# 4paradigm/OpenEmbedding

Measured on AMD Instinct MI355X. Metric: samples/sec DeepFM Criteo, higher is better.
Workload: dtype bf16; 1 GPU; model=deepfm-dim9, global_batch=4096, fields=26, dense_features=13, optimizer=adagrad, graph=True, prefetch=False, table=array, cache_mb=0, parallelism=single-gpu

## Files before the change

### openembedding_amd/models/ctr.py

```python

from __future__ import annotations

import math
from typing import List, Optional, Sequence

import torch
import torch.nn as nn

from ..ops import hip_available
from ..torch import CombinedEmbedding
from .criteo import CRITEO_FIELD_VOCABS, N_DENSE


class _FusedCTRHeadFn(torch.autograd.Function):

    @staticmethod
    def forward(ctx, e_all, dense, w, b, use_fm, out_bf16, pad32=False):
        from ..ops import require_hip
        ext = require_hip()
        wf = w.reshape(-1).contiguous()
        e_all = e_all.contiguous()
        dense = dense.contiguous()
        deep_in, partial, s = ext.ctr_head_fwd(
            e_all, dense, wf, b.reshape(-1).contiguous(), use_fm, out_bf16,
            pad32)
        ctx.save_for_backward(e_all, dense, wf, s)
        ctx.use_fm = use_fm
        return deep_in, partial

    @staticmethod
    def backward(ctx, d_deep_in, d_partial):
        from ..ops import require_hip
        ext = require_hip()
        e_all, dense, wf, s = ctx.saved_tensors
        de_all, d_dense, dw, db = ext.ctr_head_bwd(
            e_all, dense, wf, d_deep_in.contiguous(),
            d_partial.contiguous(), s, ctx.use_fm)
        return de_all, d_dense, dw.view(1, -1), db, None, None, None


class _FusedMLP3Fn(torch.autograd.Function):

    @staticmethod
    def forward(ctx, x0, partial, w1, b1, w2, b2, w3, b3, w4, b4, bufs):
        from ..ops import require_hip
        ext = require_hip()
        srcs = [w1, w2, w3]
        dsts = [bufs["w1p"], bufs["w2p"], bufs["w3p"]]
        trans = [False, False, False]
        if any(ctx.needs_input_grad) and bufs.get("grad_mode", True):
            srcs += [w3, w2, w1]
            dsts += [bufs["w3tp"], bufs["w2tp"], bufs["w1tp"]]
            trans += [True, True, True]
        ext.mlp3_pack_frag([w.contiguous() for w in srcs], dsts, trans)
        w4f = w4.reshape(-1).contiguous()
        out, a1, a2, a3 = ext.mlp3_fwd(x0, bufs["w1p"], b1, bufs["w2p"], b2,
                                       bufs["w3p"], b3, w4f, b4,
                                       None if partial is None
                                       else partial.contiguous(), frag=True)
        ctx.save_for_backward(x0, w1, w2, w3, w4f, a1, a2, a3)
        ctx.bufs = bufs
        ctx._params = (w1, b1, w2, b2, w3, b3, w4, b4)
        ctx._has_partial = partial is not None
        return out

    @staticmethod
    def backward(ctx, dout):
        from ..ops import require_hip
        ext = require_hip()
        x0, w1, w2, w3, w4f, a1, a2, a3 = ctx.saved_tensors
        bufs = ctx.bufs
        K0 = w1.shape[1]
        params = ctx._params
        prebound = all(p.grad is not None for p in params)
        bias_fused = (prebound
                      and params[1].grad.dtype == torch.bfloat16
                      and all(params[i].grad.is_contiguous()
                              for i in (1, 3, 5, 6)))
        bscratch = None
        if bias_fused:
            H0 = a1.shape[1]
            bscratch = bufs.get("bscratch")
            if bscratch is None or bscratch.numel() != 4 * H0 + 1:
                bscratch = torch.zeros(4 * H0 + 1, dtype=torch.float32,
                                       device=a1.device)
                bufs["bscratch"] = bscratch
        dx0, dz1, dz2, dz3 = ext.mlp3_bwd(
            dout.contiguous(), a1, a2, a3, w4f,
            bufs["w3tp"], bufs["w2tp"], bufs["w1tp"], bscratch, frag=True)
        def _d():
# ... 336 lines not shown
```

### openembedding_amd/ops/csrc/bindings.cpp

```cpp

#include <torch/extension.h>
#include <ATen/cuda/CUDAContext.h>
#include <c10/cuda/CUDAGuard.h>

#include <cstdint>
#include <tuple>
#include <vector>

typedef unsigned long long u64;
typedef int64_t i64;
typedef struct ihipStream_t* hipStream_t_;

extern "C" {
void emb_unique(const i64*, long, u64*, int*, long, int*, unsigned char*,
                i64*, i64*, int*, const i64*, int, hipStream_t_);
void emb_unique_indexed(const i64*, long, u64*, int*, long, int*,
                        unsigned char*, i64*, i64*, int*, const i64*, int,
                        int*, int*, int*, int*, int*, int*, int*, long, int*,
                        int*, hipStream_t_);
void emb_unique_indexed_assign(const i64*, long, u64*, int*, long, int*,
                               unsigned char*, i64*, i64*, int*, const i64*,
                               int, int*, int*, int*, int*, int*, int*, int*,
                               long, int*, int*, unsigned char*, long, long,
                               i64*, unsigned char*, hipStream_t_);
// ... 13 lines not shown
                               float*, long, const float*, hipStream_t_);
void emb_ht_lookup(u64*, int*, long, const i64*, long, int*, i64*, i64*,
                   unsigned char*, int, const int*, long, hipStream_t_);
void emb_ht_rehash(const u64*, const int*, long, u64*, int*, long,
                   hipStream_t_);
void emb_array_touch(unsigned char*, const i64*, long, long, long, i64*,
                     unsigned char*, const int*, hipStream_t_);
void emb_gather_init(float*, float*, long, long, const i64*,
                     const unsigned char*, const i64*, long, const i64*,
                     float*, int, float, float, float, u64, const float*,
                     const int*, hipStream_t_);
void emb_reduce_by_inverse(const i64*, const float*, long, long, float*, u64*,
                           long, hipStream_t_);
void emb_reduce_bags_by_inverse(const i64*, const float*, long, long,
                                const int*, const i64*, long, int, float*,
                                u64*, long, hipStream_t_);
void emb_pool_fwd(const float*, long, long, const i64*, long, const void*,
                  int, long, const i64*, long, int, float*, int*,
                  hipStream_t_);
void emb_pool_fwd_weighted(const float*, long, long, const i64*, long,
                           const void*, int, long, const i64*, long, int,
                           const float*, float*, int*, float*, hipStream_t_);
void emb_reduce_bags_weighted_by_inverse(const i64*, const float*, long, long,
                                         const int*, const float*,
                                         const float*, long, float*, u64*,
                                         long, hipStream_t_);
void emb_pool_wgrad(const float*, long, long, const i64*, long, const void*,
                    int, long, const float*, const int*, const float*,
                    const float*, const float*, long, int, float*,
                    hipStream_t_);
void emb_pool_lookup(const float*, long, long, const i64*, long, const i64*,
                     long, int, const float*, const u64*, const int*, long,
                     const unsigned char*, long, float*, hipStream_t_);
long emb_quant_stride(int, long);
void emb_quantize_rows(int, const float*, long, long, const i64*, void*,
                       long, hipStream_t_);
void emb_pool_lookup_q(int, const void*, long, long, const i64*, long,
                       const i64*, long, int, const float*, const u64*,
                       const int*, long, const unsigned char*, long, float*,
                       hipStream_t_);
void emb_gather_lookup_q(int, const void*, long, long, const i64*, long,
                         const u64*, const int*, long, const unsigned char*,
                         long, float*, hipStream_t_);
void emb_apply_optimizer(int, float*, float*, long, long, const i64*, long,
                         const float*, const u64*, const float*, const int*,
                         hipStream_t_);
void emb_ctr_head_fwd(const float*, const float*, const float*, const float*, long,
                      long, long, long, long, void*, float*, float*, int,
                      int, hipStream_t_);
void emb_ctr_head_bwd(const float*, const float*, const float*, const void*,
                      const float*, const float*, long, long, long, long,
                      long, float*, float*, float*, float*, int, int,
                      hipStream_t_);
void emb_mlp3_bias_bwd(const float*, const void*, const void*, const void*,
                       const void*, long, long, float*, void*, void*, void*,
                       void*, void*, int, int, hipStream_t_);
void emb_mlp3_wgrad(const void*, const void*, const void*, const void*,
                    const void*, const void*, long, long, long, long,
                    float*, void*, void*, void*, float*, long, hipStream_t_);
void emb_mlp3_pack(const void*, void*, long, long, long, long, int,
                   const void*, void*, long, long, long, long, int,
                   const void*, void*, long, long, long, long, int,
                   hipStream_t_);
void emb_bce_fwd(const float*, const float*, long, float*, hipStream_t_);
void emb_bce_bwd(const float*, const float*, long, const float*, float*,
                 hipStream_t_);
void emb_bucketize_pad(const i64*, long, const int*, long, long, i64*, int*,
                       int*, int*, int*, hipStream_t_);
void emb_mask_tail(i64*, float*, u64*, long, long, const int*, hipStream_t_);
void emb_mark_rows(const i64*, long, const unsigned char*, const int*,
                   const int*, int*, long, hipStream_t_);
long emb_delta_tile_rows();
long emb_delta_tiles(long);
void emb_delta_count(const int*, long, int, const int*, const unsigned char*,
                     int*, hipStream_t_);
void emb_delta_compact(const int*, long, int, const int*,
                       const unsigned char*, const int*, i64*, hipStream_t_);
void emb_delta_gather(const float*, const float*, long, long, long,
                      const i64*, long, long, const i64*, long, long, long,
                      const int*, i64*, float*, float*, hipStream_t_);
void emb_fault_in(const i64*, long, const int*, const u64*, const int*, long,
                  const float*, const float*, float*, float*, long, long,
                  const i64*, unsigned char*, int*, hipStream_t_);
void emb_spill_rows(const i64*, const i64*, long, const float*, const float*,
                    float*, float*, long, long, hipStream_t_);
void emb_gather_host(const i64*, long, const i64*, const u64*, const int*,
                     long, const float*, float*, long, hipStream_t_);
void emb_gather_pad(const float*, const u64*, long, const int*, long, float*,
                    hipStream_t_);
void emb_scatter_out(const float*, const i64*, long, const int*, long, float*,
                     hipStream_t_);
void emb_split_payload(const float*, long, long, const int*, float*, u64*,
                       hipStream_t_);
void emb_flat_step_scalars(float*, float, float, hipStream_t_);
void emb_flat_opt(int, void*, float*, float*, float*, void*,
                  const float*, long, int, float, float, float, float,
                  hipStream_t_);
void emb_flat_adagrad_f32(float*, float*, const float*, long, float, float,
                          hipStream_t_);
void emb_flat_adagrad_bf16(float*, float*, const void*, void*, long, float,
                           float, hipStream_t_);
void emb_cin_fwd(const float*, const float*, const void*, float*, long,
                 long, long, long, long, hipStream_t_);
void emb_cin_dw(const void*, const void*, const void*, float*, long, long,
                long, long, long, hipStream_t_);
void emb_cin_dx(const float*, const void*, const float*, const float*,
// ... 1092 lines not shown
    return send_p;
}

torch::Tensor scatter_out(torch::Tensor rows_recv, torch::Tensor inverse,
                          torch::Tensor pos_of, int64_t n_elems) {
    CHECK_GPU(rows_recv); CHECK_CONT(rows_recv); CHECK_CONT(inverse);
    CHECK_CONT(pos_of);
    TORCH_CHECK(rows_recv.dtype() == torch::kFloat32 &&
                pos_of.dtype() == torch::kInt32, "scatter_out dtypes");
    const c10::cuda::CUDAGuard guard(rows_recv.device());
    long dim = rows_recv.size(1);
    auto out = torch::empty({n_elems, dim}, rows_recv.options());
    emb_scatter_out(rows_recv.data_ptr<float>(), inverse.data_ptr<i64>(),
                    n_elems, pos_of.data_ptr<int>(), dim,
                    out.data_ptr<float>(), cur_stream());
    return out;
}

std::tuple<torch::Tensor, torch::Tensor> split_payload(torch::Tensor g2c,
                                                       OptTensor u_dev) {
    CHECK_GPU(g2c); CHECK_CONT(g2c);
    TORCH_CHECK(g2c.dtype() == torch::kFloat32, "split_payload dtype");
    const c10::cuda::CUDAGuard guard(g2c.device());
    long u = g2c.size(0);
    long dim = g2c.size(1) - 1;
    auto grads = torch::empty({u, dim}, g2c.options());
    auto counts = torch::empty({u}, g2c.options().dtype(torch::kInt64));
    emb_split_payload(g2c.data_ptr<float>(), u, dim, u_ptr(u_dev),
                      grads.data_ptr<float>(), (u64*)counts.data_ptr<i64>(),
                      cur_stream());
    return {grads, counts};
}


void apply_optimizer(int64_t opt, torch::Tensor weights, torch::Tensor state,
                     torch::Tensor slots, torch::Tensor grads,
                     torch::Tensor counts, std::vector<double> cfg,
                     OptTensor u_dev) {
    CHECK_GPU(weights); CHECK_CONT(weights); CHECK_CONT(grads);
    const c10::cuda::CUDAGuard guard(weights.device());
    long n = slots.numel();
    long dim = weights.size(1);
    long sd = state.numel() ? state.size(1) : 0;
    float c[7] = {0, 0, 0, 0, 0, 0, 0};
    for (size_t i = 0; i < cfg.size() && i < 7; ++i) c[i] = (float)cfg[i];
    emb_apply_optimizer((int)opt, weights.data_ptr<float>(),
                        sd ? state.data_ptr<float>() : nullptr, dim, sd,
                        slots.data_ptr<i64>(), n, grads.data_ptr<float>(),
                        (const u64*)counts.data_ptr<i64>(), c, u_ptr(u_dev),
                        cur_stream());
}


std::tuple<torch::Tensor, torch::Tensor, torch::Tensor> ctr_head_fwd(
    torch::Tensor e_all, torch::Tensor dense, torch::Tensor w,
    torch::Tensor bias, bool use_fm, bool out_bf16, bool pad32) {
    CHECK_GPU(e_all); CHECK_CONT(e_all); CHECK_CONT(dense); CHECK_CONT(w);
    const c10::cuda::CUDAGuard guard(e_all.device());
    long B = e_all.size(0), F = e_all.size(1), D1 = e_all.size(2);
    long dim = D1 - 1, nd = dense.size(1);
    TORCH_CHECK(D1 <= 128, "ctr_head: dim+1 must be <= 128");
    TORCH_CHECK(nd <= 32, "ctr_head: dense features must be <= 32");
    auto out_opts = e_all.options().dtype(out_bf16 ? torch::kBFloat16
                                                   : torch::kFloat32);
    long width = F * dim + nd;
    long stride = pad32 ? ((width + 31) / 32) * 32 : width;
    auto deep_in = torch::empty({B, stride}, out_opts);
    auto partial = torch::empty({B}, e_all.options());
    auto s_out = torch::empty({B, dim}, e_all.options());
    CHECK_CONT(bias);
    emb_ctr_head_fwd(e_all.data_ptr<float>(), dense.data_ptr<float>(),
                     w.data_ptr<float>(), bias.data_ptr<float>(), B, F, dim, nd,
                     stride, deep_in.data_ptr(), partial.data_ptr<float>(),
                     s_out.data_ptr<float>(),
                     use_fm ? 1 : 0, out_bf16 ? 1 : 0, cur_stream());
    return {deep_in, partial, s_out};
}

std::tuple<torch::Tensor, torch::Tensor, torch::Tensor, torch::Tensor>
ctr_head_bwd(torch::Tensor e_all, torch::Tensor dense, torch::Tensor w,
             torch::Tensor d_deep_in, torch::Tensor d_partial,
             torch::Tensor s_in, bool use_fm) {
    CHECK_GPU(e_all); CHECK_CONT(e_all); CHECK_CONT(d_deep_in);
    const c10::cuda::CUDAGuard guard(e_all.device());
    long B = e_all.size(0), F = e_all.size(1), D1 = e_all.size(2);
    long dim = D1 - 1, nd = dense.size(1);
    long stride = d_deep_in.size(1);
    bool out_bf16 = d_deep_in.dtype() == torch::kBFloat16;
    auto de_all = torch::empty_like(e_all);
    auto d_dense = torch::empty_like(dense);
    auto dw = torch::empty_like(w);
    auto db = torch::empty({1}, w.options());
    if (B == 0) { dw.zero_(); db.zero_(); }
    emb_ctr_head_bwd(e_all.data_ptr<float>(), dense.data_ptr<float>(),
                     w.data_ptr<float>(), d_deep_in.data_ptr(),
                     d_partial.data_ptr<float>(),
                     s_in.data_ptr<float>(), B, F, dim, nd, stride,
                     de_all.data_ptr<float>(), d_dense.data_ptr<float>(),
                     dw.data_ptr<float>(), db.data_ptr<float>(),
                     use_fm ? 1 : 0, out_bf16 ? 1 : 0, cur_stream());
    return {de_all, d_dense, dw, db};
}


void flat_adagrad(torch::Tensor param, torch::Tensor accum,
                  torch::Tensor grad, c10::optional<torch::Tensor> master,
                  double lr, double eps) {
    CHECK_GPU(param); CHECK_CONT(param); CHECK_CONT(accum); CHECK_CONT(grad);
    const c10::cuda::CUDAGuard guard(param.device());
    long n = param.numel();
    if (param.dtype() == torch::kFloat32) {
        emb_flat_adagrad_f32(param.data_ptr<float>(), accum.data_ptr<float>(),
                             grad.data_ptr<float>(), n, (float)lr, (float)eps,
                             cur_stream());
    } else {
        TORCH_CHECK(param.dtype() == torch::kBFloat16 && master.has_value(),
                    "bf16 flat_adagrad needs a float32 master tensor");
        emb_flat_adagrad_bf16(master->data_ptr<float>(),
                              accum.data_ptr<float>(), grad.data_ptr(),
                              param.data_ptr(), n, (float)lr, (float)eps,
                              cur_stream());
    }
}

void flat_step_scalars(torch::Tensor sc, double b1, double b2) {
    CHECK_GPU(sc); CHECK_CONT(sc);
    TORCH_CHECK(sc.numel() >= 3 && sc.dtype() == torch::kFloat32,
                "step scalars must be float32 [3]");
    const c10::cuda::CUDAGuard guard(sc.device());
    emb_flat_step_scalars(sc.data_ptr<float>(), (float)b1, (float)b2,
                          cur_stream());
}

void flat_opt(int64_t opt, torch::Tensor param, OptTensor master,
              OptTensor s1, OptTensor s2, torch::Tensor grad, OptTensor sc,
              double lr, double c0, double c1, double c2) {
    CHECK_GPU(param); CHECK_CONT(param); CHECK_CONT(grad);
    const c10::cuda::CUDAGuard guard(param.device());
    long n = param.numel();
    bool bf16 = param.dtype() == torch::kBFloat16;
    float* mp = nullptr;
    if (bf16) {
        TORCH_CHECK(master.has_value(), "bf16 flat_opt needs fp32 master");
        mp = master->data_ptr<float>();
    } else {
        TORCH_CHECK(param.dtype() == torch::kFloat32, "flat_opt dtype");
    }
    emb_flat_opt((int)opt, param.data_ptr(), mp,
                 s1.has_value() ? s1->data_ptr<float>() : nullptr,
                 s2.has_value() ? s2->data_ptr<float>() : nullptr,
                 grad.data_ptr(),
                 sc.has_value() ? sc->data_ptr<float>() : nullptr,
                 n, bf16 ? 1 : 0, (float)lr, (float)c0, (float)c1,
                 (float)c2, cur_stream());
// ... 399 lines not shown
          "flat read over a packed slab, keys -> fp32 rows in one launch",
          pybind11::arg("slab"), pybind11::arg("dim"), pybind11::arg("fmt"),
          pybind11::arg("keys"),
          pybind11::arg("tk") = pybind11::none(),
          pybind11::arg("tv") = pybind11::none(),
          pybind11::arg("valid") = pybind11::none(),
          pybind11::arg("shard_num") = 1);
    m.def("apply_optimizer", &apply_optimizer, "fused sparse optimizer step");
    m.def("mask_tail", &mask_tail,
          "zero the garbage tail of a bounded block (enables multi-block "
          "merge by concatenation)");
    m.def("mark_rows", &mark_rows,
          "delta checkpoints: row_epoch[slot] = *epoch_dev for the named "
          "rows (optional byte mask and device count)",
          pybind11::arg("slots"), pybind11::arg("mask") = pybind11::none(),
          pybind11::arg("u_dev") = pybind11::none(),
          pybind11::arg("epoch_dev"), pybind11::arg("row_epoch"));
    m.attr("DELTA_TILE_ROWS") = emb_delta_tile_rows();
    m.def("select_changed", &select_changed,
          "delta checkpoints: ascending slots of the live rows with "
          "row_epoch >= since -> (slots [R] with a -1 tail, n_dev int32[1])",
          pybind11::arg("row_epoch"), pybind11::arg("since"),
          pybind11::arg("nrows_dev") = pybind11::none(),
          pybind11::arg("valid") = pybind11::none());
    m.def("gather_rows_by_slot", &gather_rows_by_slot,
          "delta checkpoints: keys, weights and state of "
          "slots[start:start+count] into staging buffers",
          pybind11::arg("weights"), pybind11::arg("state"),
          pybind11::arg("slot_keys") = pybind11::none(),
          pybind11::arg("shard_num") = 1, pybind11::arg("shard_id") = 0,
          pybind11::arg("slots"), pybind11::arg("start"),
          pybind11::arg("count"), pybind11::arg("n_dev"),
          pybind11::arg("keys_out") = pybind11::none(),
          pybind11::arg("w_out") = pybind11::none(),
          pybind11::arg("s_out") = pybind11::none());
    m.def("fault_in", &fault_in,
          "tier v2: copy host-resident rows into fresh cache slots, "
          "clearing their lazy-init mask");
    m.def("spill_rows", &spill_rows,
          "tier v2: copy cache rows into the pinned host slab");
    m.def("gather_host", &gather_host,
          "tier v2: read-only host-row gather for cache misses");
    m.def("bucketize_pad", &bucketize_pad,
          "owner-bucketize unique keys into a fixed padded [world, cap] "
          "wire block (sync-free multi-rank route)");
    m.def("gather_pad", &gather_pad,
          "gather grads+counts payload into the padded send layout");
    m.def("scatter_out", &scatter_out,
          "padded pull: wire rows -> per-element output (fused dup scatter)");
    m.def("split_payload", &split_payload,
          "split owner-reduced payload into grads + int64 counts");
    m.def("ctr_head_fwd", &ctr_head_fwd,
          "fused CTR head fwd: deep_in assembly (+cast) + FM + first-order "
          "+ dense linear");
    m.def("ctr_head_bwd", &ctr_head_bwd, "fused CTR head backward");
    m.def("mlp3_bwd", &mlp3_bwd,
          "fused dgrad chain backward of the 3-layer MLP (optionally "
          "carrying the head wgrad/bias sums)",
          pybind11::arg("dout"), pybind11::arg("a1"), pybind11::arg("a2"),
          pybind11::arg("a3"), pybind11::arg("w4"), pybind11::arg("w3t"),
          pybind11::arg("w2t"), pybind11::arg("w1t"),
          pybind11::arg("bias_scratch") = pybind11::none(),
          pybind11::arg("bm") = 0, pybind11::arg("frag") = false);
    m.def("mlp3_pack", &mlp3_pack,
          "refresh three padded (or transposed) weight copies in one "
          "launch");
    m.def("mlp3_pack_frag", &mlp3_pack_frag,
          "write up to six fragment-major weight images (pads included) "
          "in one launch",
          pybind11::arg("srcs"), pybind11::arg("dsts"),
          pybind11::arg("trans"));
    m.def("mlp3_fwd", &mlp3_fwd,
          "fused 3-hidden-layer MLP forward (bf16 MFMA, bias+ReLU fused)",
          pybind11::arg("x0"), pybind11::arg("w1"), pybind11::arg("b1"),
          pybind11::arg("w2"), pybind11::arg("b2"), pybind11::arg("w3"),
          pybind11::arg("b3"), pybind11::arg("w4"), pybind11::arg("b4"),
          pybind11::arg("partial"), pybind11::arg("bm") = 0,
          pybind11::arg("frag") = false);
    m.def("mlp3_wgrad", &mlp3_wgrad,
          pybind11::arg("dz1"), pybind11::arg("dz2"), pybind11::arg("dz3"),
          pybind11::arg("x0"), pybind11::arg("a1"), pybind11::arg("a2"),
          pybind11::arg("scratch"), pybind11::arg("dw1"),
          pybind11::arg("dw2"), pybind11::arg("dw3"),
          pybind11::arg("bias_scratch") = pybind11::none(),
          pybind11::arg("m_split") = 0,
          "all three MLP weight grads in one MFMA launch (+= into bf16 "
          "grads via fp32 scratch)");
    m.def("mlp3_bias_bwd", &mlp3_bias_bwd,
          "MLP bias grads + head wgrad in one pass over the dz mirrors "
          "(with_dz=false when the fused wgrad carried the dz sums)",
          pybind11::arg("dout"), pybind11::arg("dz1"), pybind11::arg("dz2"),
          pybind11::arg("dz3"), pybind11::arg("a3"),
          pybind11::arg("scratch"), pybind11::arg("db1"),
          pybind11::arg("db2"), pybind11::arg("db3"), pybind11::arg("dw4"),
          pybind11::arg("db4"), pybind11::arg("with_dz") = true,
          pybind11::arg("with_head") = true);
    m.def("cin_fwd", &cin_fwd,
          "CIN layer forward: implicit outer-product MFMA GEMM");
    m.def("cin_dw", &cin_dw,
          "CIN weight grad: per-field split-K MFMA with on-the-fly operand");
    m.def("cin_dx", &cin_dx,
          "CIN input grads: P=W^T dZ GEMM fused with the xk/x0 contractions");
    m.def("bce_fwd", &bce_fwd, "fused BCE-with-logits forward (mean)");
    m.def("bce_bwd", &bce_bwd, "fused BCE-with-logits backward");
    m.def("flat_adagrad", &flat_adagrad,
          "fused flat-buffer Adagrad (f32, or bf16 weights + f32 master)");
    m.def("flat_opt", &flat_opt,
          "fused flat-buffer dense optimizer (0=sgd, 1=adagrad, 2=adam)");
// ... 5 lines not shown
```

### openembedding_amd/ops/csrc/ctrhead.hip

```cpp

#include <hip/hip_runtime.h>
#include <hip/hip_bf16.h>
#include <cstdint>

typedef long long i64;
typedef unsigned long long u64;
typedef __hip_bfloat16 bf16;

template <typename OutT>
__global__ void k_ctr_head_fwd(const float* __restrict__ e_all,
                               const float* __restrict__ dense,
                               const float* __restrict__ w,
                               const float* __restrict__ bias,
                               long B, long F, long dim, long nd,
                               long out_stride,
                               OutT* __restrict__ deep_in,
                               float* __restrict__ partial,
                               float* __restrict__ s_out,
                               int use_fm) {
    const long D1 = dim + 1;
    const int lane = threadIdx.x & 63;
    const long b = ((long)blockIdx.x * blockDim.x + threadIdx.x) >> 6;
    if (b >= B) return;
    const float* e = e_all + b * F * D1;
// ... 49 lines not shown
                                 long B, long F, long dim,
                                 long nd, long out_stride,
                                 float* __restrict__ de_all,
                                 int use_fm,
                                 float* __restrict__ dw,
                                 float* __restrict__ db) {
    const long D1 = dim + 1;
    long i = (long)blockIdx.x * blockDim.x + threadIdx.x;
    if (i < nd) dw[i] = 0.0f;
    if (i == nd) *db = 0.0f;
    if (i >= B * F * D1) return;
    const long c = i % D1;
    const long f = (i / D1) % F;
    const long b = i / (D1 * F);
    const float gp = d_partial[b];
    if (c == dim) { de_all[i] = gp; return; }
    float g = (float)d_deep_in[b * out_stride + f * dim + c];
    if (use_fm) g += gp * (s_in[b * dim + c] - e_all[i]);
    de_all[i] = g;
}

#define ND_MAX 32
template <typename OutT>
__global__ void k_ctr_head_bwd_d(const float* __restrict__ dense,
                                 const float* __restrict__ w,
                                 const OutT* __restrict__ d_deep_in,
                                 const float* __restrict__ d_partial,
                                 long B, long F, long dim, long nd,
                                 long out_stride,
                                 float* __restrict__ d_dense,
                                 float* __restrict__ dw,
                                 float* __restrict__ db) {
    __shared__ float lacc[ND_MAX + 1];
    for (int t = threadIdx.x; t < nd + 1; t += blockDim.x) lacc[t] = 0.0f;
    __syncthreads();
    long i = (long)blockIdx.x * blockDim.x + threadIdx.x;
    if (i < B * nd) {
        const long b = i / nd;
        const long j = i % nd;
        const float gp = d_partial[b];
        const float dv = dense[i];
        d_dense[i] = (float)d_deep_in[b * out_stride + F * dim + j]
                     + gp * w[j];
        atomicAdd(&lacc[j], gp * dv);
        if (j == 0) atomicAdd(&lacc[nd], gp);
    }
    __syncthreads();
    for (int t = threadIdx.x; t < nd + 1; t += blockDim.x) {
        if (t < nd) atomicAdd(&dw[t], lacc[t]);
        else atomicAdd(db, lacc[nd]);
    }
}

extern "C" {

void emb_ctr_head_fwd(const float* e_all, const float* dense, const float* w,
                      const float* bias, long B, long F, long dim, long nd,
                      long out_stride, void* deep_in, float* partial,
                      float* s_out, int use_fm, int out_bf16,
                      hipStream_t stream) {
    if (B == 0) return;
    int block = 256;
    long grid = (B * 64 + block - 1) / block;
    if (out_bf16)
        k_ctr_head_fwd<bf16><<<(int)grid, block, 0, stream>>>(
            e_all, dense, w, bias, B, F, dim, nd, out_stride,
            (bf16*)deep_in, partial, s_out, use_fm);
    else
        k_ctr_head_fwd<float><<<(int)grid, block, 0, stream>>>(
            e_all, dense, w, bias, B, F, dim, nd, out_stride,
            (float*)deep_in, partial, s_out, use_fm);
}

void emb_ctr_head_bwd(const float* e_all, const float* dense, const float* w,
                      const void* d_deep_in, const float* d_partial,
                      const float* s_in,
                      long B, long F, long dim, long nd, long out_stride,
                      float* de_all, float* d_dense, float* dw, float* db,
                      int use_fm, int out_bf16, hipStream_t stream) {
    if (B == 0) return;
    int block = 256;
    long grid_e = (B * F * (dim + 1) + block - 1) / block;
    long grid_d = (B * nd + block - 1) / block;
    if (out_bf16) {
        k_ctr_head_bwd_e<bf16><<<(int)grid_e, block, 0, stream>>>(
            e_all, (const bf16*)d_deep_in, d_partial, s_in, B, F, dim, nd,
            out_stride, de_all, use_fm, dw, db);
        k_ctr_head_bwd_d<bf16><<<(int)grid_d, block, 0, stream>>>(
            dense, w, (const bf16*)d_deep_in, d_partial, B, F, dim, nd,
            out_stride, d_dense, dw, db);
    } else {
        k_ctr_head_bwd_e<float><<<(int)grid_e, block, 0, stream>>>(
            e_all, (const float*)d_deep_in, d_partial, s_in, B, F, dim, nd,
            out_stride, de_all, use_fm, dw, db);
        k_ctr_head_bwd_d<float><<<(int)grid_d, block, 0, stream>>>(
            dense, w, (const float*)d_deep_in, d_partial, B, F, dim, nd,
            out_stride, d_dense, dw, db);
    }
}

}
```

Before: 19.93 million samples/s.

## Add LDS row-staged CTR head kernels and fuse backward dw/db into grads

Adds forward and backward CTR-head kernels in which each wave handles one sample. A block's rows of e_all and deep_in are staged through LDS with vectorized 16-byte copies so global accesses are coalesced, replacing the element-wise scattered accesses of the old kernels. The backward kernel is persistent and folds the e, dense and dw/db reductions into one launch. When the parameter grads already exist, it accumulates dw/db straight into them, skipping temporary allocation and the autograd add. This adds a lot of kernel complexity, large LDS use that limits occupancy, and an env switch that defaults to on.

```diff
diff --git a/openembedding_amd/models/ctr.py b/openembedding_amd/models/ctr.py
--- a/openembedding_amd/models/ctr.py
+++ b/openembedding_amd/models/ctr.py
@@ -2,6 +2,7 @@
 from __future__ import annotations
 
 import math
+import os
 from typing import List, Optional, Sequence
 
 import torch
@@ -10,6 +11,12 @@
 from ..ops import hip_available
 from ..torch import CombinedEmbedding
 from .criteo import CRITEO_FIELD_VOCABS, N_DENSE
+
+
+_HEAD_ROWS_ENV = os.environ.get("OEAMD_HEAD_ROWS", "1")
+_HEAD_ROWS = _HEAD_ROWS_ENV != "0"
+_HEAD_ROWS_FWD = _HEAD_ROWS_ENV not in ("0", "bwd")
+_HEAD_ROWS_BWD = _HEAD_ROWS_ENV not in ("0", "fwd")
 
 
 class _FusedCTRHeadFn(torch.autograd.Function):
@@ -23,9 +30,10 @@
         dense = dense.contiguous()
         deep_in, partial, s = ext.ctr_head_fwd(
             e_all, dense, wf, b.reshape(-1).contiguous(), use_fm, out_bf16,
-            pad32)
+            pad32, 0 if _HEAD_ROWS_FWD else 1)
         ctx.save_for_backward(e_all, dense, wf, s)
         ctx.use_fm = use_fm
+        ctx._params = (w, b)
         return deep_in, partial
 
     @staticmethod
@@ -33,9 +41,22 @@
         from ..ops import require_hip
         ext = require_hip()
         e_all, dense, wf, s = ctx.saved_tensors
+        w, b = ctx._params
+        prebound = _HEAD_ROWS_BWD and all(
+            p.requires_grad and p.grad is not None
+            and p.grad.dtype == torch.float32
+            and p.grad.is_contiguous() and p.grad.device == e_all.device
+            for p in (w, b))
+        if prebound:
+            de_all, d_dense = ext.ctr_head_bwd_acc(
+                e_all, dense, wf, d_deep_in.contiguous(),
+                d_partial.contiguous(), s, ctx.use_fm, w.grad.view(-1),
+                b.grad.view(-1), ctx.needs_input_grad[1])
+            return de_all, d_dense, None, None, None, None, None
         de_all, d_dense, dw, db = ext.ctr_head_bwd(
             e_all, dense, wf, d_deep_in.contiguous(),
-            d_partial.contiguous(), s, ctx.use_fm)
+            d_partial.contiguous(), s, ctx.use_fm,
+            0 if _HEAD_ROWS_BWD else 1)
         return de_all, d_dense, dw.view(1, -1), db, None, None, None
 
 
diff --git a/openembedding_amd/ops/csrc/bindings.cpp b/openembedding_amd/ops/csrc/bindings.cpp
--- a/openembedding_amd/ops/csrc/bindings.cpp
+++ b/openembedding_amd/ops/csrc/bindings.cpp
@@ -89,6 +89,15 @@
                       const float*, const float*, long, long, long, long,
                       long, float*, float*, float*, float*, int, int,
                       hipStream_t_);
+int emb_ctr_head_rows_waves(long, long, long, long, long, int, int);
+long emb_ctr_head_rows_bwd_grid(long, long, int);
+void emb_ctr_head_fwd_rows(const float*, const float*, const float*,
+                           const float*, long, long, long, long, long, void*,
+                           float*, float*, int, int, int, hipStream_t_);
+void emb_ctr_head_bwd_rows(const float*, const float*, const float*,
+                           const void*, const float*, const float*, long,
+                           long, long, long, long, float*, float*, float*,
+                           float*, int, int, int, hipStream_t_);
 void emb_mlp3_bias_bwd(const float*, const void*, const void*, const void*,
                        const void*, long, long, float*, void*, void*, void*,
                        void*, void*, int, int, hipStream_t_);
@@ -1287,10 +1296,14 @@
 }
 
 
+#define CHECK_F32(t) \
+    TORCH_CHECK((t).scalar_type() == torch::kFloat32, #t " must be float32")
+
 std::tuple<torch::Tensor, torch::Tensor, torch::Tensor> ctr_head_fwd(
     torch::Tensor e_all, torch::Tensor dense, torch::Tensor w,
-    torch::Tensor bias, bool use_fm, bool out_bf16, bool pad32) {
+    torch::Tensor bias, bool use_fm, bool out_bf16, bool pad32, int64_t impl) {
     CHECK_GPU(e_all); CHECK_CONT(e_all); CHECK_CONT(dense); CHECK_CONT(w);
+    TORCH_CHECK(impl >= 0 && impl <= 2, "ctr_head: impl must be 0, 1 or 2");
     const c10::cuda::CUDAGuard guard(e_all.device());
     long B = e_all.size(0), F = e_all.size(1), D1 = e_all.size(2);
     long dim = D1 - 1, nd = dense.size(1);
@@ -1300,30 +1313,104 @@
                                                    : torch::kFloat32);
     long width = F * dim + nd;
     long stride = pad32 ? ((width + 31) / 32) * 32 : width;
+    int S = 0;
+    if (impl != 1) {
+        S = emb_ctr_head_rows_waves(B, F, dim, nd, stride, out_bf16 ? 1 : 0,
+                                    0);
+        TORCH_CHECK(S > 0 || impl == 0, "ctr_head_fwd: impl 2, but the "
+                    "row-staged kernel does not fit this shape");
+    }
+    if (S > 0) {
+        CHECK_F32(e_all); CHECK_F32(dense); CHECK_F32(w); CHECK_F32(bias);
+        CHECK_GPU(dense); CHECK_GPU(w); CHECK_GPU(bias);
+        TORCH_CHECK(dense.size(0) == B && w.numel() == nd
+                    && bias.numel() >= 1, "ctr_head_fwd: operand lengths");
+    }
     auto deep_in = torch::empty({B, stride}, out_opts);
     auto partial = torch::empty({B}, e_all.options());
     auto s_out = torch::empty({B, dim}, e_all.options());
     CHECK_CONT(bias);
-    emb_ctr_head_fwd(e_all.data_ptr<float>(), dense.data_ptr<float>(),
-                     w.data_ptr<float>(), bias.data_ptr<float>(), B, F, dim, nd,
-                     stride, deep_in.data_ptr(), partial.data_ptr<float>(),
-                     s_out.data_ptr<float>(),
-                     use_fm ? 1 : 0, out_bf16 ? 1 : 0, cur_stream());
+    if (S > 0)
+        emb_ctr_head_fwd_rows(e_all.data_ptr<float>(),
+                              dense.data_ptr<float>(), w.data_ptr<float>(),
+                              bias.data_ptr<float>(), B, F, dim, nd, stride,
+                              deep_in.data_ptr(), partial.data_ptr<float>(),
+                              s_out.data_ptr<float>(), use_fm ? 1 : 0,
+                              out_bf16 ? 1 : 0, S, cur_stream());
+    else
+        emb_ctr_head_fwd(e_all.data_ptr<float>(), dense.data_ptr<float>(),
+                         w.data_ptr<float>(), bias.data_ptr<float>(), B, F,
+                         dim, nd, stride, deep_in.data_ptr(),
+                         partial.data_ptr<float>(), s_out.data_ptr<float>(),
+                         use_fm ? 1 : 0, out_bf16 ? 1 : 0, cur_stream());
     return {deep_in, partial, s_out};
+}
+
+static bool head_bwd_check(const torch::Tensor& e_all,
+                           const torch::Tensor& dense,
+                           const torch::Tensor& w,
+                           const torch::Tensor& d_deep_in,
+                           const torch::Tensor& d_partial,
+                           const torch::Tensor& s_in) {
+    CHECK_GPU(e_all); CHECK_GPU(dense); CHECK_GPU(w); CHECK_GPU(d_deep_in);
+    CHECK_GPU(d_partial); CHECK_GPU(s_in);
+    CHECK_CONT(e_all); CHECK_CONT(dense); CHECK_CONT(w);
+    CHECK_CONT(d_deep_in); CHECK_CONT(d_partial); CHECK_CONT(s_in);
+    CHECK_F32(e_all); CHECK_F32(dense); CHECK_F32(w); CHECK_F32(d_partial);
+    CHECK_F32(s_in);
+    TORCH_CHECK(e_all.dim() == 3 && dense.dim() == 2 && d_deep_in.dim() == 2,
+                "ctr_head_bwd: e_all [B,F,D1], dense [B,nd], d_deep_in "
+                "[B,stride]");
+    long B = e_all.size(0), F = e_all.size(1), dim = e_all.size(2) - 1;
+    long nd = dense.size(1);
+    bool bf = d_deep_in.scalar_type() == torch::kBFloat16;
+    TORCH_CHECK(bf || d_deep_in.scalar_type() == torch::kFloat32,
+                "ctr_head_bwd: d_deep_in must be bfloat16 or float32");
+    TORCH_CHECK(dense.size(0) == B && w.numel() == nd
+                && d_deep_in.size(0) == B
+                && d_deep_in.size(1) >= F * dim + nd
+                && d_partial.numel() == B && s_in.numel() == B * dim,
+                "ctr_head_bwd: operand lengths");
+    return bf;
 }
 
 std::tuple<torch::Tensor, torch::Tensor, torch::Tensor, torch::Tensor>
 ctr_head_bwd(torch::Tensor e_all, torch::Tensor dense, torch::Tensor w,
              torch::Tensor d_deep_in, torch::Tensor d_partial,
-             torch::Tensor s_in, bool use_fm) {
+             torch::Tensor s_in, bool use_fm, int64_t impl) {
     CHECK_GPU(e_all); CHECK_CONT(e_all); CHECK_CONT(d_deep_in);
+    TORCH_CHECK(impl >= 0 && impl <= 2, "ctr_head: impl must be 0, 1 or 2");
     const c10::cuda::CUDAGuard guard(e_all.device());
     long B = e_all.size(0), F = e_all.size(1), D1 = e_all.size(2);
     long dim = D1 - 1, nd = dense.size(1);
     long stride = d_deep_in.size(1);
     bool out_bf16 = d_deep_in.dtype() == torch::kBFloat16;
+    int S = 0;
+    if (impl != 1) {
+        S = emb_ctr_head_rows_waves(B, F, dim, nd, stride, out_bf16 ? 1 : 0,
+                                    impl == 0 ? 2 : 1);
+        TORCH_CHECK(S > 0 || impl == 0, "ctr_head_bwd: impl 2, but the "
+                    "row-staged kernel does not fit this shape");
+    }
     auto de_all = torch::empty_like(e_all);
     auto d_dense = torch::empty_like(dense);
+    if (S > 0) {
+        head_bwd_check(e_all, dense, w, d_deep_in, d_partial, s_in);
+        auto acc = torch::zeros({nd + 1}, w.options());
+        auto dw = acc.narrow(0, 0, nd).view_as(w);
+        auto db = acc.narrow(0, nd, 1);
+        emb_ctr_head_bwd_rows(e_all.data_ptr<float>(),
+                              dense.data_ptr<float>(), w.data_ptr<float>(),
+                              d_deep_in.data_ptr(),
+                              d_partial.data_ptr<float>(),
+                              s_in.data_ptr<float>(), B, F, dim, nd, stride,
+                              de_all.data_ptr<float>(),
+                              d_dense.data_ptr<float>(),
+                              dw.data_ptr<float>(), db.data_ptr<float>(),
+                              use_fm ? 1 : 0, out_bf16 ? 1 : 0, S,
+                              cur_stream());
+        return {de_all, d_dense, dw, db};
+    }
     auto dw = torch::empty_like(w);
     auto db = torch::empty({1}, w.options());
     if (B == 0) { dw.zero_(); db.zero_(); }
@@ -1335,6 +1422,59 @@
                      dw.data_ptr<float>(), db.data_ptr<float>(),
                      use_fm ? 1 : 0, out_bf16 ? 1 : 0, cur_stream());
     return {de_all, d_dense, dw, db};
+}
+
+std::tuple<torch::Tensor, c10::optional<torch::Tensor>>
+ctr_head_bwd_acc(torch::Tensor e_all, torch::Tensor dense, torch::Tensor w,
+                 torch::Tensor d_deep_in, torch::Tensor d_partial,
+                 torch::Tensor s_in, bool use_fm, torch::Tensor dw_acc,
+                 torch::Tensor db_acc, bool want_d_dense) {
+    bool out_bf16 = head_bwd_check(e_all, dense, w, d_deep_in, d_partial,
+                                   s_in);
+    long B = e_all.size(0), F = e_all.size(1), dim = e_all.size(2) - 1;
+    long nd = dense.size(1), stride = d_deep_in.size(1);
+    CHECK_GPU(dw_acc); CHECK_GPU(db_acc); CHECK_CONT(dw_acc);
+    CHECK_CONT(db_acc); CHECK_F32(dw_acc); CHECK_F32(db_acc);
+    TORCH_CHECK(dw_acc.dim() == 1 && dw_acc.numel() == nd,
+                "ctr_head_bwd_acc: dw_acc must be [nd]");
+    TORCH_CHECK(db_acc.dim() == 1 && db_acc.numel() == 1,
+                "ctr_head_bwd_acc: db_acc must be [1]");
+    TORCH_CHECK(dw_acc.device() == e_all.device()
+                && db_acc.device() == e_all.device(),
+                "ctr_head_bwd_acc: accumulators on another device");
+    const c10::cuda::CUDAGuard guard(e_all.device());
+    int S = emb_ctr_head_rows_waves(B, F, dim, nd, stride, out_bf16 ? 1 : 0,
+                                    2);
+    if (S == 0) {
+        auto r = ctr_head_bwd(e_all, dense, w, d_deep_in, d_partial, s_in,
+                              use_fm, 1);
+        dw_acc.add_(std::get<2>(r).reshape(-1));
+        db_acc.add_(std::get<3>(r));
+        if (want_d_dense) return {std::get<0>(r), std::get<1>(r)};
+        return {std::get<0>(r), c10::nullopt};
+    }
+    auto de_all = torch::empty_like(e_all);
+    c10::optional<torch::Tensor> d_dense;
+    if (want_d_dense) d_dense = torch::empty_like(dense);
+    emb_ctr_head_bwd_rows(e_all.data_ptr<float>(), dense.data_ptr<float>(),
+                          w.data_ptr<float>(), d_deep_in.data_ptr(),
+                          d_partial.data_ptr<float>(),
+                          s_in.data_ptr<float>(), B, F, dim, nd, stride,
+                          de_all.data_ptr<float>(),
+                          want_d_dense ? d_dense->data_ptr<float>() : nullptr,
+                          dw_acc.data_ptr<float>(),
+                          db_acc.data_ptr<float>(), use_fm ? 1 : 0,
+                          out_bf16 ? 1 : 0, S, cur_stream());
+    return {de_all, d_dense};
+}
+
+std::tuple<int64_t, int64_t, int64_t, bool> ctr_head_rows_plan(
+    int64_t B, int64_t F, int64_t dim, int64_t nd, int64_t stride,
+    bool out_bf16) {
+    int sf = emb_ctr_head_rows_waves(B, F, dim, nd, stride, out_bf16, 0);
+    int sb = emb_ctr_head_rows_waves(B, F, dim, nd, stride, out_bf16, 1);
+    int sa = emb_ctr_head_rows_waves(B, F, dim, nd, stride, out_bf16, 2);
+    return {sf, sb, sb ? emb_ctr_head_rows_bwd_grid(B, nd, sb) : 0, sa > 0};
 }
 
 
@@ -1840,8 +1980,26 @@
           "split owner-reduced payload into grads + int64 counts");
     m.def("ctr_head_fwd", &ctr_head_fwd,
           "fused CTR head fwd: deep_in assembly (+cast) + FM + first-order "
-          "+ dense linear");
-    m.def("ctr_head_bwd", &ctr_head_bwd, "fused CTR head backward");
+          "+ dense linear",
+          pybind11::arg("e_all"), pybind11::arg("dense"), pybind11::arg("w"),
+          pybind11::arg("bias"), pybind11::arg("use_fm"),
+          pybind11::arg("out_bf16"), pybind11::arg("pad32"),
+          pybind11::arg("impl") = 0);
+    m.def("ctr_head_bwd", &ctr_head_bwd, "fused CTR head backward",
+          pybind11::arg("e_all"), pybind11::arg("dense"), pybind11::arg("w"),
+          pybind11::arg("d_deep_in"), pybind11::arg("d_partial"),
+          pybind11::arg("s"), pybind11::arg("use_fm"),
+          pybind11::arg("impl") = 0);
+    m.def("ctr_head_bwd_acc", &ctr_head_bwd_acc,
+          "fused CTR head backward in one launch, dw/db added into the "
+          "caller's buffers",
+          pybind11::arg("e_all"), pybind11::arg("dense"), pybind11::arg("w"),
+          pybind11::arg("d_deep_in"), pybind11::arg("d_partial"),
+          pybind11::arg("s"), pybind11::arg("use_fm"),
+          pybind11::arg("dw_acc"), pybind11::arg("db_acc"),
+          pybind11::arg("want_d_dense") = true);
+    m.def("ctr_head_rows_plan", &ctr_head_rows_plan,
+          "samples per block of the row-staged head kernels for a shape");
     m.def("mlp3_bwd", &mlp3_bwd,
           "fused dgrad chain backward of the 3-layer MLP (optionally "
           "carrying the head wgrad/bias sums)",
diff --git a/openembedding_amd/ops/csrc/ctrhead.hip b/openembedding_amd/ops/csrc/ctrhead.hip
--- a/openembedding_amd/ops/csrc/ctrhead.hip
+++ b/openembedding_amd/ops/csrc/ctrhead.hip
@@ -125,6 +125,324 @@
     }
 }
 
+
+#define ROWS_U 4
+#define ROWS_LDS_MAX 65280
+
+template <int ESZ>
+__device__ __forceinline__ void rows_copy_edges(const char* src, char* dst,
+                                                int lo, int hi, int q_lo,
+                                                int q_hi) {
+    const int head_end = min(16 * q_lo, hi);
+    const int tail = max(16 * q_hi, head_end);
+    const int t = threadIdx.x * ESZ;
+    if (lo + t < head_end) {
+        if (ESZ == 4)
+            *(uint32_t*)(dst + lo + t) = *(const uint32_t*)(src + lo + t);
+        else
+            *(uint16_t*)(dst + lo + t) = *(const uint16_t*)(src + lo + t);
+    }
+    if (tail + t < hi) {
+        if (ESZ == 4)
+            *(uint32_t*)(dst + tail + t) = *(const uint32_t*)(src + tail + t);
+        else
+            *(uint16_t*)(dst + tail + t) = *(const uint16_t*)(src + tail + t);
+    }
+}
+
+__device__ __forceinline__ void rows_load(const char* g0, int n_full, int i0,
+                                          uint4 (&v)[ROWS_U]) {
+    const int i_blk = i0 - threadIdx.x;
+    const int bd = blockDim.x;
+    #pragma unroll
+    for (int u = 0; u < ROWS_U; ++u) {
+        v[u] = make_uint4(0, 0, 0, 0);
+        if (i_blk + u * bd < n_full)
+            v[u] = *(const uint4*)(g0 + 16 * min(i0 + u * bd, n_full - 1));
+    }
+}
+
+__device__ __forceinline__ void rows_hold(uint4 (&v)[ROWS_U]) {
+    #pragma unroll
+    for (int u = 0; u < ROWS_U; ++u)
+        asm volatile("" : "+v"(v[u].x), "+v"(v[u].y), "+v"(v[u].z),
+                     "+v"(v[u].w));
+}
+
+__device__ __forceinline__ void rows_store(char* l0, int n_full, int i0,
+                                           const uint4 (&v)[ROWS_U]) {
+    const int bd = blockDim.x;
+    #pragma unroll
+    for (int u = 0; u < ROWS_U; ++u)
+        if (i0 + u * bd < n_full)
+            *(uint4*)(l0 + 16 * (i0 + u * bd)) = v[u];
+}
+
+template <int ESZ>
+__device__ __forceinline__ void rows_stage_in(const char* gb, char* lds,
+                                              int lo, int hi) {
+    const int q_lo = (lo + 15) >> 4, q_hi = hi >> 4;
+    const int n_full = q_hi - q_lo;
+    for (int i0 = threadIdx.x; i0 < n_full; i0 += ROWS_U * blockDim.x) {
+        uint4 v[ROWS_U];
+        rows_load(gb + 16 * q_lo, n_full, i0, v);
+        rows_hold(v);
+        rows_store(lds + 16 * q_lo, n_full, i0, v);
+    }
+    rows_copy_edges<ESZ>(gb, lds, lo, hi, q_lo, q_hi);
+}
+
+template <int ESZ_A, int ESZ_B>
+__device__ __forceinline__ void rows_stage_in2(const char* gb_a, char* lds_a,
+                                               int lo_a, int hi_a,
+                                               const char* gb_b, char* lds_b,
+                                               int lo_b, int hi_b) {
+    const int qa = (lo_a + 15) >> 4, na = (hi_a >> 4) - qa;
+    const int qb = (lo_b + 15) >> 4, nb = (hi_b >> 4) - qb;
+    for (int i0 = threadIdx.x; i0 < max(na, nb);
+         i0 += ROWS_U * blockDim.x) {
+        uint4 va[ROWS_U], vb[ROWS_U];
+        rows_load(gb_a + 16 * qa, na, i0, va);
+        rows_load(gb_b + 16 * qb, nb, i0, vb);
+        rows_hold(va);
+        rows_hold(vb);
+        rows_store(lds_a + 16 * qa, na, i0, va);
+        rows_store(lds_b + 16 * qb, nb, i0, vb);
+    }
+    rows_copy_edges<ESZ_A>(gb_a, lds_a, lo_a, hi_a, qa, hi_a >> 4);
+    rows_copy_edges<ESZ_B>(gb_b, lds_b, lo_b, hi_b, qb, hi_b >> 4);
+}
+
+template <int ESZ>
+__device__ __forceinline__ void rows_stage_out(const char* lds, char* gb,
+                                               int lo, int hi) {
+    const int q_lo = (lo + 15) >> 4, q_hi = hi >> 4;
+    for (int q = q_lo + threadIdx.x; q < q_hi; q += blockDim.x)
+        *(uint4*)(gb + 16 * q) = *(const uint4*)(lds + 16 * q);
+    rows_copy_edges<ESZ>(lds, gb, lo, hi, q_lo, q_hi);
+}
+
+template <typename OutT>
+__global__ void k_ctr_head_fwd_rows(const float* __restrict__ e_all,
+                                    const float* __restrict__ dense,
+                                    const float* __restrict__ w,
+                                    const float* __restrict__ bias,
+                                    int B, int F, int dim, int nd,
+                                    int out_stride,
+                                    OutT* __restrict__ deep_in,
+                                    float* __restrict__ partial,
+                                    float* __restrict__ s_out,
+                                    int use_fm, int img_b, int p_shift) {
+    extern __shared__ uint4 rows_smem[];
+    char* const img_e = (char*)rows_smem;
+    char* const img_o = img_e + img_b;
+    const int S = blockDim.x >> 6;
+    const int lane = threadIdx.x & 63, wave = threadIdx.x >> 6;
+    const int D1 = dim + 1, R = F * D1;
+    const int c0 = p_shift < 6 ? lane & ((1 << p_shift) - 1) : lane;
+    const int f_first = p_shift < 6 ? lane >> p_shift : 0;
+    const int f_step = p_shift < 6 ? 64 >> p_shift : 1;
+    const int b0 = blockIdx.x * S;
+    const int n = min(S, B - b0);
+    const float* ge = e_all + (size_t)b0 * R;
+    OutT* go = deep_in + (size_t)b0 * out_stride;
+    const int mis_e = (int)((uintptr_t)ge & 15);
+    const int mis_o = (int)((uintptr_t)go & 15);
+    const int b = b0 + wave;
+    const bool live = wave < n;
+
+    float dv = 0.0f, wv = 0.0f;
+    if (live && lane < nd) {
+        dv = dense[(size_t)b * nd + lane];
+        wv = w[lane];
+    }
+    rows_stage_in<4>((const char*)ge - mis_e, img_e, mis_e,
+                     mis_e + n * R * 4);
+    __syncthreads();
+
+    if (live) {
+        const float* e = (const float*)(img_e + mis_e) + wave * R;
+        OutT* o = (OutT*)(img_o + mis_o) + wave * out_stride;
+        float s[2] = {0.0f, 0.0f}, sq[2] = {0.0f, 0.0f};
+        #pragma unroll
+        for (int t = 0; t < 2; ++t) {
+            const int cc = lane + 64 * t;
+            if (cc >= D1) break;
+            const bool emb = cc < dim;
+            for (int f0 = 0; f0 < F; f0 += 8) {
+                float v[8];
+                #pragma unroll
+                for (int u = 0; u < 8; ++u)
+                    v[u] = e[min(f0 + u, F - 1) * D1 + cc];
+                #pragma unroll
+                for (int u = 0; u < 8; ++u) {
+                    if (f0 + u >= F) break;
+                    s[t] += v[u];
+                    if (emb) sq[t] += v[u] * v[u];
+                }
+            }
+        }
+        #pragma unroll
+        for (int t = 0; t < 2; ++t) {
+            const int c = c0 + 64 * t;
+            if (c >= dim) break;
+            for (int f = f_first; f < F; f += 4 * f_step) {
+                float v[4];
+                #pragma unroll
+                for (int u = 0; u < 4; ++u)
+                    v[u] = e[min(f + u * f_step, F - 1) * D1 + c];
+                #pragma unroll
+                for (int u = 0; u < 4; ++u)
+                    if (f + u * f_step < F)
+                        o[(f + u * f_step) * dim + c] = (OutT)v[u];
+            }
+        }
+        float dsum = 0.0f;
+        if (lane < nd) {
+            o[F * dim + lane] = (OutT)dv;
+            dsum += dv * wv;
+        }
+        for (int j = F * dim + nd + lane; j < out_stride; j += 64)
+            o[j] = (OutT)0.0f;
+        float fm = 0.0f, lin = 0.0f;
+        #pragma unroll
+        for (int t = 0; t < 2; ++t) {
+            const int cc = lane + 64 * t;
+            if (cc >= D1) break;
+            if (cc < dim) {
+                if (use_fm) fm += s[t] * s[t] - sq[t];
+                if (s_out) s_out[(size_t)b * dim + cc] = s[t];
+            } else {
+                lin = s[t];
+            }
+        }
+        float acc = 0.5f * fm + lin + dsum;
+        for (int off = 32; off; off >>= 1)
+            acc += __shfl_down(acc, off, 64);
+        if (lane == 0) partial[b] = acc + bias[0];
+    }
+    __syncthreads();
+    rows_stage_out<(int)sizeof(OutT)>(img_o, (char*)go - mis_o, mis_o,
+                                      mis_o + n * out_stride
+                                      * (int)sizeof(OutT));
+}
+
+template <typename OutT>
+__global__ void k_ctr_head_bwd_rows(const float* __restrict__ e_all,
+                                    const float* __restrict__ dense,
+                                    const float* __restrict__ w,
+                                    const OutT* __restrict__ d_deep_in,
+                                    const float* __restrict__ d_partial,
+                                    const float* __restrict__ s_in,
+                                    int B, int F, int dim, int nd,
+                                    int out_stride,
+                                    float* __restrict__ de_all,
+                                    float* __restrict__ d_dense,
+                                    float* __restrict__ dw,
+                                    float* __restrict__ db,
+                                    int use_fm, int img_b, int p_shift,
+                                    int n_groups) {
+    extern __shared__ uint4 rows_smem[];
+    __shared__ float lacc[ND_MAX + 1];
+    char* const img_e = (char*)rows_smem;
+    char* const img_d = img_e + img_b;
+    const int S = blockDim.x >> 6;
+    const int lane = threadIdx.x & 63, wave = threadIdx.x >> 6;
+    const int D1 = dim + 1, R = F * D1;
+    const int c0 = p_shift < 6 ? lane & ((1 << p_shift) - 1) : lane;
+    const int f_first = p_shift < 6 ? lane >> p_shift : 0;
+    const int f_step = p_shift < 6 ? 64 >> p_shift : 1;
+    for (int t = threadIdx.x; t < nd + 1; t += blockDim.x) lacc[t] = 0.0f;
+
+    for (int g = blockIdx.x; g < n_groups; g += gridDim.x) {
+        if (g != (int)blockIdx.x) __syncthreads();
+        const int b0 = g * S;
+        const int n = min(S, B - b0);
+        const float* ge = e_all + (size_t)b0 * R;
+        const OutT* gd = d_deep_in + (size_t)b0 * out_stride;
+        float* gde = de_all + (size_t)b0 * R;
+        const int mis_e = (int)((uintptr_t)ge & 15);
+        const int mis_d = (int)((uintptr_t)gd & 15);
+        const int mis_de = (int)((uintptr_t)gde & 15);
+        const int b = b0 + wave;
+        const bool live = wave < n;
+
+        float gp = 0.0f, dv = 0.0f, wv = 0.0f, sv[2] = {0.0f, 0.0f};
+        if (live) {
+            gp = d_partial[b];
+            if (lane < nd) {
+                dv = dense[(size_t)b * nd + lane];
+                wv = w[lane];
+            }
+            if (use_fm) {
+                #pragma unroll
+                for (int t = 0; t < 2; ++t)
+                    if (c0 + 64 * t < dim)
+                        sv[t] = s_in[(size_t)b * dim + c0 + 64 * t];
+            }
+        }
+        const int hi_d = mis_d + n * out_stride * (int)sizeof(OutT);
+        if (mis_e == mis_de) {
+            rows_stage_in2<4, (int)sizeof(OutT)>(
+                (const char*)ge - mis_e, img_e, mis_e, mis_e + n * R * 4,
+                (const char*)gd - mis_d, img_d, mis_d, hi_d);
+        } else {
+            float* e = (float*)(img_e + mis_de);
+            for (int i = threadIdx.x; i < n * R; i += blockDim.x)
+                e[i] = ge[i];
+            rows_stage_in<(int)sizeof(OutT)>((const char*)gd - mis_d, img_d,
+                                             mis_d, hi_d);
+        }
+        __syncthreads();
+
+        if (live) {
+            float* e = (float*)(img_e + mis_de) + wave * R;
+            const OutT* d = (const OutT*)(img_d + mis_d) + wave * out_stride;
+            #pragma unroll
+            for (int t = 0; t < 2; ++t) {
+                const int c = c0 + 64 * t;
+                if (c >= D1) break;
+                for (int f = f_first; f < F; f += 4 * f_step) {
+                    float dv4[4], ev[4];
+                    #pragma unroll
+                    for (int u = 0; u < 4; ++u) {
+                        const int fu = min(f + u * f_step, F - 1);
+                        dv4[u] = (float)d[fu * dim + c];
+                        ev[u] = e[fu * D1 + c];
+                    }
+                    #pragma unroll
+                    for (int u = 0; u < 4; ++u) {
+                        if (f + u * f_step >= F) break;
+                        const int i = (f + u * f_step) * D1 + c;
+                        if (c == dim) {
+                            e[i] = gp;
+                        } else {
+                            float gv = dv4[u];
+                            if (use_fm) gv += gp * (sv[t] - ev[u]);
+                            e[i] = gv;
+                        }
+                    }
+                }
+            }
+            if (lane < nd) {
+                if (d_dense)
+                    d_dense[(size_t)b * nd + lane] =
+                        (float)d[F * dim + lane] + gp * wv;
+                atomicAdd(&lacc[lane], gp * dv);
+            }
+            if (lane == 0) atomicAdd(&lacc[nd], gp);
+        }
+        __syncthreads();
+        rows_stage_out<4>(img_e, (char*)gde - mis_de, mis_de,
+                          mis_de + n * R * 4);
+    }
+    __syncthreads();
+    for (int t = threadIdx.x; t < nd + 1; t += blockDim.x) {
+        if (t < nd) atomicAdd(&dw[t], lacc[t]);
+        else atomicAdd(db, lacc[nd]);
+    }
+}
+
 extern "C" {
 
 void emb_ctr_head_fwd(const float* e_all, const float* dense, const float* w,
@@ -172,4 +490,82 @@
     }
 }
 
-}
+
+static long rows_img_bytes(long S, long row_bytes) {
+    return (S * row_bytes + 15) / 16 * 16 + 16;
+}
+
+static int rows_p_shift(long D1) {
+    int p_shift = 0;
+    while ((1L << p_shift) < D1) ++p_shift;
+    return p_shift;
+}
+
+int emb_ctr_head_rows_waves(long B, long F, long dim, long nd,
+                            long out_stride, int out_bf16, int bwd) {
+    const long D1 = dim + 1, R = F * D1, osz = out_bf16 ? 2 : 4;
+    if (nd < 1 || nd > ND_MAX || dim < 0 || D1 > 128 || F < 1) return 0;
+    if (B * R >= (1L << 31) || B * out_stride >= (1L << 31)) return 0;
+    for (int S = bwd ? 16 : 4; S >= 1; S >>= 1)
+        if (rows_img_bytes(S, R * 4) + rows_img_bytes(S, out_stride * osz)
+            <= ROWS_LDS_MAX)
+            return bwd == 2 && S < 16 ? 0 : S;
+    return 0;
+}
+
+long emb_ctr_head_rows_bwd_grid(long B, long nd, int S) {
+    const long groups = (B + S - 1) / S;
+    const long cap = (B * nd + 255) / 256;
+    return groups < cap ? groups : (cap < 1 ? 1 : cap);
+}
+
+void emb_ctr_head_fwd_rows(const float* e_all, const float* dense,
+                           const float* w, const float* bias, long B, long F,
+                           long dim, long nd, long out_stride, void* deep_in,
+                           float* partial, float* s_out, int use_fm,
+                           int out_bf16, int S, hipStream_t stream) {
+    if (B == 0) return;
+    const long img_b = rows_img_bytes(S, F * (dim + 1) * 4);
+    const long lds = img_b + rows_img_bytes(S, out_stride
+                                            * (out_bf16 ? 2 : 4));
+    const long grid = (B + S - 1) / S;
+    const int p_shift = rows_p_shift(dim + 1);
+    if (out_bf16)
+        k_ctr_head_fwd_rows<bf16><<<(int)grid, 64 * S, lds, stream>>>(
+            e_all, dense, w, bias, (int)B, (int)F, (int)dim, (int)nd,
+            (int)out_stride, (bf16*)deep_in, partial, s_out, use_fm,
+            (int)img_b, p_shift);
+    else
+        k_ctr_head_fwd_rows<float><<<(int)grid, 64 * S, lds, stream>>>(
+            e_all, dense, w, bias, (int)B, (int)F, (int)dim, (int)nd,
+            (int)out_stride, (float*)deep_in, partial, s_out, use_fm,
+            (int)img_b, p_shift);
+}
+
+void emb_ctr_head_bwd_rows(const float* e_all, const float* dense,
+                           const float* w, const void* d_deep_in,
+                           const float* d_partial, const float* s_in,
+                           long B, long F, long dim, long nd,
+                           long out_stride, float* de_all, float* d_dense,
+                           float* dw, float* db, int use_fm, int out_bf16,
+                           int S, hipStream_t stream) {
+    if (B == 0) return;
+    const long img_b = rows_img_bytes(S, F * (dim + 1) * 4);
+    const long lds = img_b + rows_img_bytes(S, out_stride
+                                            * (out_bf16 ? 2 : 4));
+    const long groups = (B + S - 1) / S;
+    const long grid = emb_ctr_head_rows_bwd_grid(B, nd, S);
+    const int p_shift = rows_p_shift(dim + 1);
+    if (out_bf16)
+        k_ctr_head_bwd_rows<bf16><<<(int)grid, 64 * S, lds, stream>>>(
+            e_all, dense, w, (const bf16*)d_deep_in, d_partial, s_in,
+            (int)B, (int)F, (int)dim, (int)nd, (int)out_stride, de_all,
+            d_dense, dw, db, use_fm, (int)img_b, p_shift, (int)groups);
+    else
+        k_ctr_head_bwd_rows<float><<<(int)grid, 64 * S, lds, stream>>>(
+            e_all, dense, w, (const float*)d_deep_in, d_partial, s_in,
+            (int)B, (int)F, (int)dim, (int)nd, (int)out_stride, de_all,
+            d_dense, dw, db, use_fm, (int)img_b, p_shift, (int)groups);
+}
+
+}
```

Result: faster. 21.15 million samples/s, median of 6 (+6.1%).
